# UCL/gp_emulator

Hardware: AMD Instinct MI355X
Metric: test-points/sec for predict(mean+var+grad), N_train=250 D=11 (higher is better)
Workload: dtype f64

## Files before the change

### gp_emulator_amd/csrc/gp_predict_kernel.hpp

```cpp
#pragma once
#include <hip/hip_runtime.h>
#include <stdint.h>
#include <type_traits>
#include <utility>

namespace gpk {

#ifndef GP_WAVES
#define GP_WAVES 8
#endif
#ifndef GP_WAVES_F32
#define GP_WAVES_F32 12
#endif
#ifndef GP_CHUNK
#define GP_CHUNK 64
#endif
#ifndef GP_CHUNK_F32
#define GP_CHUNK_F32 192
#endif
#ifndef GP_ABLATE
#define GP_ABLATE 0
#endif
#ifndef GP_AHEAD
#define GP_AHEAD 4
#endif
#ifndef GP_AHEAD_F32
#define GP_AHEAD_F32 8
#endif
#ifndef GP_RING_PIN
#define GP_RING_PIN 1
#endif
#ifndef GP_MU_DOUBLE
#define GP_MU_DOUBLE 1
#endif
#ifndef GP_ESTRIN
#define GP_ESTRIN 0
#endif
#ifndef GP_DOTSPLIT
#define GP_DOTSPLIT 1
#endif
#ifndef GP_GROUP_F64
#define GP_GROUP_F64 1
#endif
#ifndef GP_STAMPS
#define GP_STAMPS 0
#endif
constexpr int kTile = 16;
template <typename T, bool kVar = true> struct Geo {
  static constexpr int kWaves = sizeof(T) == 8 ? GP_WAVES : GP_WAVES_F32;
  static constexpr int kThreads = kWaves * 64;
#ifndef GP_WG_PER_CU_SMALL
#define GP_WG_PER_CU_SMALL 0
#endif
  static constexpr int kWGPerCU = kWaves >= 8 ? 1 : (GP_WG_PER_CU_SMALL > 0 ? GP_WG_PER_CU_SMALL : 8 / kWaves);
  static constexpr int kWavesPerSimd = kWaves >= 8 ? kWaves / 4 : kWGPerCU * kWaves / 4;
  static constexpr int kRowsPerWG = kWaves * kTile;
  static constexpr int kChunk = sizeof(T) == 8 ? GP_CHUNK : GP_CHUNK_F32;
};
#ifndef GP_MG_WAVES
#define GP_MG_WAVES 12
#endif
#ifndef GP_MG_WAVES_F32
#define GP_MG_WAVES_F32 16
#endif
#ifndef GP_MG_WG_PER_CU
#define GP_MG_WG_PER_CU 1
#endif
template <typename T> struct Geo<T, false> {
  static constexpr int kWaves = sizeof(T) == 8 ? GP_MG_WAVES : GP_MG_WAVES_F32;
  static constexpr int kThreads = kWaves * 64;
  static constexpr int kWGPerCU = GP_MG_WG_PER_CU;
  static constexpr int kWavesPerSimd = kWGPerCU * kWaves / 4;
  static constexpr int kRowsPerWG = kWaves * kTile;
  static constexpr int kChunk = 1;
};

typedef double f64x4 __attribute__((ext_vector_type(4)));
typedef float f32x4 __attribute__((ext_vector_type(4)));

template <typename F, int... Is>
__device__ __forceinline__ void static_for_impl(F&& f, std::integer_sequence<int, Is...>) {
  (f(std::integral_constant<int, Is>{}), ...);
}
template <int N, typename F>
__device__ __forceinline__ void static_for(F&& f) {
  static_for_impl(f, std::make_integer_sequence<int, N>{});
}

template <typename T> struct Real;
template <> struct Real<double> {
  typedef f64x4 acc_t;
  static constexpr bool kExpand = true;
  static constexpr int kGroup = GP_GROUP_F64;
  __host__ __device__ static constexpr int own_sub(int r, int g) { return 4 * r + g; }
  __device__ static inline acc_t mfma(double a, double b, acc_t c) {
    return __builtin_amdgcn_mfma_f64_16x16x4f64(a, b, c, 0, 0, 0);
  }
  __device__ static inline double exp_(double x) {
    x = __builtin_fmax(x, -1000.0);
    const double n = __builtin_rint(x * 1.4426950408889634);
    double r = fma(n, -6.93147180559945286e-01, x);
    r = fma(n, -2.31904681384629956e-17, r);
#if GP_ESTRIN
    const double r2 = r * r;
    const double p01 = fma(1.00000000000000666e+00, r, 1.0);
    const double p23 = fma(1.66666666665544028e-01, r, 5.00000000000000555e-01);
    const double p45 = fma(8.33333338566834801e-03, r, 4.16666666665732183e-02);
    const double p67 = fma(1.98411702695461072e-04, r, 1.38888889324666632e-03);
    const double p89 = fma(2.76401812311866076e-06, r, 2.48015043709117912e-05);
    const double r4 = r2 * r2;
    const double q0 = fma(r2, p23, p01);
    const double q1 = fma(r2, p67, p45);
    const double q2 = fma(r2, 2.76263485910095559e-07, p89);
    const double r8 = r4 * r4;
    const double s0 = fma(r4, q1, q0);
    const double p = fma(r8, q2, s0);
#else
    double p = 2.76263485910095559e-07;
    p = fma(p, r, 2.76401812311866076e-06);
    p = fma(p, r, 2.48015043709117912e-05);
    p = fma(p, r, 1.98411702695461072e-04);
    p = fma(p, r, 1.38888889324666632e-03);
    p = fma(p, r, 8.33333338566834801e-03);
    p = fma(p, r, 4.16666666665732183e-02);
    p = fma(p, r, 1.66666666665544028e-01);
    p = fma(p, r, 5.00000000000000555e-01);
    p = fma(p, r, 1.00000000000000666e+00);
    p = fma(p, r, 1.0);
#endif
    return ldexp(p, (int)n);
  }
  template <int GP>
  __device__ static inline void exp_n(double (&x)[GP]) {
    double n[GP], r[GP], p[GP];
#pragma unroll
    for (int u = 0; u < GP; ++u) x[u] = __builtin_fmax(x[u], -1000.0);
#pragma unroll
    for (int u = 0; u < GP; ++u) n[u] = __builtin_rint(x[u] * 1.4426950408889634);
#pragma unroll
    for (int u = 0; u < GP; ++u) r[u] = fma(n[u], -6.93147180559945286e-01, x[u]);
#pragma unroll
    for (int u = 0; u < GP; ++u) r[u] = fma(n[u], -2.31904681384629956e-17, r[u]);
#pragma unroll
    for (int u = 0; u < GP; ++u) p[u] = 2.76263485910095559e-07;
    constexpr double c[10] = {2.76401812311866076e-06, 2.48015043709117912e-05, 1.98411702695461072e-04,
                              1.38888889324666632e-03, 8.33333338566834801e-03, 4.16666666665732183e-02,
                              1.66666666665544028e-01, 5.00000000000000555e-01, 1.00000000000000666e+00, 1.0};
#pragma unroll
    for (int j = 0; j < 10; ++j) {
#pragma unroll
      for (int u = 0; u < GP; ++u) p[u] = fma(p[u], r[u], c[j]);
    }
#pragma unroll
    for (int u = 0; u < GP; ++u) x[u] = ldexp(p[u], (int)n[u]);
  }
};
template <> struct Real<float> {
  typedef f32x4 acc_t;
  static constexpr bool kExpand = false;
#ifndef GP_GROUP_F32
#define GP_GROUP_F32 2
#endif
  static constexpr int kGroup = GP_GROUP_F32;
  __host__ __device__ static constexpr int own_sub(int r, int g) { return 4 * g + r; }
  __device__ static inline acc_t mfma(float a, float b, acc_t c) {
    return __builtin_amdgcn_mfma_f32_16x16x4f32(a, b, c, 0, 0, 0);
  }
  __device__ static inline float exp_(float x) { return __expf(x); }
  template <int GP>
  __device__ static inline void exp_n(float (&x)[GP]) {
#pragma unroll
    for (int u = 0; u < GP; ++u) x[u] = __expf(x[u]);
  }
};

template <typename T>
__host__ __device__ constexpr int own_index(int I, int s, int g) {
  return 16 * I + Real<T>::own_sub(s, g);
}

template <typename T>
__host__ __device__ constexpr int point_slot(int n) {
  return 16 * (n / 16) + Real<T>::own_sub((n % 16) / 4, n % 4);
}
template <typename T>
__host__ __device__ constexpr int slot_point(int slot) {
  for (int q = 0; q < 16; ++q)
    if (Real<T>::own_sub(q / 4, q % 4) == slot % 16) return 16 * (slot / 16) + q;
  return -1;
}

struct FragId { int I, J, s; };
__host__ __device__ constexpr int frag_count(int NB) { return NB * (NB + 1) / 2 * 4; }
__host__ __device__ constexpr int frag_col_offset(int J, int NB) { return J * NB - J * (J - 1) / 2; }
__host__ __device__ constexpr FragId frag_at(int n, int NB) {
  const int pair = n >> 2;
  int J = 0;
  while (J + 1 < NB && frag_col_offset(J + 1, NB) <= pair) ++J;
  return FragId{J + pair - frag_col_offset(J, NB), J, n & 3};
}
__host__ __device__ constexpr int frag_index(int I, int J, int s, int NB) {
  return (frag_col_offset(J, NB) + (I - J)) * 4 + s;
}
__host__ __device__ constexpr int frag_count_padded(int NB, int chunk) {
  return (frag_count(NB) + chunk - 1) / chunk * chunk;
}

__host__ __device__ constexpr int row_stride(int D) { return (D + 2 + 3) & ~3; }
#ifndef GP_XA_PAD
#define GP_XA_PAD 1
#endif
template <typename T> __host__ __device__ constexpr int xa_lds_stride(int D) {
  return (GP_XA_PAD && sizeof(T) == 4 && row_stride(D) % 16 == 0) ? row_stride(D) + 4 : row_stride(D);
}

template <typename T>
struct PredictArgs {
  const T* xa;
  const T* frags;
  const T* sd;
  const T* testing;
  T* mu;
  T* var;
  T* deriv;
  long long M;
  int d_actual;
  int deriv_row_major;
  int n_emulators;
  long long xa_stride, frags_stride, sd_stride;
  unsigned long long* dbg;
  int rows_prescaled;
};

template <int XOR>
__device__ __forceinline__ unsigned swap_halves(unsigned x, unsigned& other) {
  if constexpr (XOR == 16) {
    auto r = __builtin_amdgcn_permlane16_swap(x, x, false, false);
    other = r[1];
    return r[0];
  } else {
    auto r = __builtin_amdgcn_permlane32_swap(x, x, false, false);
    other = r[1];
    return r[0];
  }
}
template <int XOR>
__device__ __forceinline__ float pair_sum(float v) {
  unsigned o, a = swap_halves<XOR>(__float_as_uint(v), o);
  return __uint_as_float(a) + __uint_as_float(o);
}
template <int XOR>
__device__ __forceinline__ double pair_sum(double v) {
  const unsigned long long u = (unsigned long long)__double_as_longlong(v);
  unsigned lo_o, hi_o;
  const unsigned lo_a = swap_halves<XOR>((unsigned)u, lo_o);
  const unsigned hi_a = swap_halves<XOR>((unsigned)(u >> 32), hi_o);
  const double a = __longlong_as_double((long long)(((unsigned long long)hi_a << 32) | lo_a));
  const double o = __longlong_as_double((long long)(((unsigned long long)hi_o << 32) | lo_o));
  return a + o;
}

template <typename T, int N>
__device__ inline void xor_reduce_groups_n(T* v) {
#pragma unroll
  for (int i = 0; i < N; ++i) v[i] = pair_sum<32>(pair_sum<16>(v[i]));
}

template <typename T>
__device__ inline T xor_reduce_groups(T v) {
  return pair_sum<32>(pair_sum<16>(v));
}

template <typename T, int kWaves = Geo<T>::kWaves, int kChunk = Geo<T>::kChunk>
__device__ __forceinline__ void stage_chunk(const T* src, T* dst, int wave, int lane) {
  constexpr int kBytes = kChunk * 64 * (int)sizeof(T);
  constexpr int kPieces = kBytes / 1024;
  static_assert(kPieces * 1024 == kBytes, "chunk must be whole 1 KiB pieces");
  const unsigned voff = (unsigned)lane * 16u;
  const unsigned lds0 = (unsigned)(uintptr_t)(
      (__attribute__((address_space(3))) char*)(reinterpret_cast<char*>(dst)));
#pragma unroll
  for (int pc0 = 0; pc0 < kPieces; pc0 += kWaves) {
    const int pc = pc0 + wave;
    if (pc0 + kWaves <= kPieces || pc < kPieces) {
      const char* s = reinterpret_cast<const char*>(src) + pc * 1024;
      const unsigned m0v = __builtin_amdgcn_readfirstlane(lds0 + pc * 1024);
      unsigned keep;
      asm volatile(
          "s_mov_b32 %0, m0\n\t"
          "s_mov_b32 m0, %1\n\t"
          "s_nop 4\n\t"
          "global_load_lds_dwordx4 %2, %3\n\t"
          "s_mov_b32 m0, %0"
          : "=&s"(keep)
          : "s"(m0v), "v"(voff), "s"(s)
          : "memory");
    }
  }
}
template <typename T, int NP>
__device__ __forceinline__ void stage_pieces(const T* src, T* dst, int first_piece, int lane) {
  const unsigned voff = (unsigned)lane * 16u;
  const unsigned lds0 = (unsigned)(uintptr_t)(
      (__attribute__((address_space(3))) char*)(reinterpret_cast<char*>(dst)));
#pragma unroll
  for (int i = 0; i < NP; ++i) {
    const int pc = first_piece + i;
    const char* s = reinterpret_cast<const char*>(src) + pc * 1024;
    const unsigned m0v = __builtin_amdgcn_readfirstlane(lds0 + pc * 1024);
    unsigned keep;
    asm volatile(
        "s_mov_b32 %0, m0\n\t"
        "s_mov_b32 m0, %1\n\t"
        "s_nop 4\n\t"
        "global_load_lds_dwordx4 %2, %3\n\t"
        "s_mov_b32 m0, %0"
        : "=&s"(keep)
        : "s"(m0v), "v"(voff), "s"(s)
        : "memory");
  }
}
__device__ __forceinline__ void dma_wait() { asm volatile("s_waitcnt vmcnt(0)" ::: "memory"); }

#if GP_STAMPS == 1
#define GP_STAMP(seg)                                                                    \
  do {                                                                                   \
    __builtin_amdgcn_sched_barrier(0);                                                   \
    unsigned long long now_;                                                             \
    asm volatile("s_memtime %0\n\ts_waitcnt lgkmcnt(0)" : "=s"(now_)::"memory");         \
    __builtin_amdgcn_sched_barrier(0);                                                   \
    seg_sum[seg] += now_ - seg_t0;                                                       \
    seg_t0 = now_;                                                                       \
  } while (0)
#else
#define GP_STAMP(seg) do { } while (0)
#endif

template <typename T, int D, int NK, bool kVar = true>
__global__ __launch_bounds__((Geo<T, kVar>::kThreads), (Geo<T, kVar>::kWavesPerSimd)) void predict_kernel(PredictArgs<T> p) {
  typedef Real<T> R;
  typedef Geo<T, kVar> G;
  constexpr int kThreads = G::kThreads;
  constexpr int kRowsPerWG = G::kRowsPerWG;
  typedef typename R::acc_t acc_t;
  constexpr int NB = (NK + 3) / 4;
  constexpr int KL = NK - 4 * (NB - 1);
  constexpr int NP = 16 * NB;
  constexpr int DSG = row_stride(D);
  constexpr int DS = xa_lds_stride<T>(D);
  constexpr int NF = frag_count(NB);
  constexpr int kChunk = G::kChunk;
  constexpr int NCH = (NF + kChunk - 1) / kChunk;

  __shared__ __attribute__((aligned(16))) T s_xa[NP * DS];
  __shared__ __attribute__((aligned(16))) T s_fr[kVar ? 2 : 1][kVar ? kChunk * 64 : 1];
  __shared__ T s_sd[2 * D + 1];
  __shared__ T s_ts[2 * D];
  __shared__ T s_rows[2][G::kWaves][kTile * D];

  const int tid = threadIdx.x;
  const int lane = tid & 63;
  const int wave = __builtin_amdgcn_readfirstlane(tid >> 6);
  const int ml = lane & 15;
  const int g = lane >> 4;

  const int n_groups = (int)((p.M + kRowsPerWG - 1) / kRowsPerWG);
  int e = 0, cur_e = -1;
  int grp = blockIdx.x;
  while (grp >= n_groups && e < p.n_emulators) { grp -= n_groups; ++e; }

  constexpr int NJ = (kTile * D + 63) / 64;
  auto fetch_rows = [&](int grp_, T (&regs)[NJ]) {
    const long long e0 = ((long long)grp_ * kRowsPerWG + wave * kTile) * p.d_actual;
    const long long emax = p.M * p.d_actual - 1;
#pragma unroll
    for (int j = 0; j < NJ; ++j) {
      long long e_ = e0 + lane + 64 * j;
      e_ = e_ < emax ? e_ : emax;
      regs[j] = p.testing[e_];
    }
  };
  auto stash_rows = [&](int buf_, const T (&regs)[NJ]) {
#pragma unroll
    for (int j = 0; j < NJ; ++j)
      if (lane + 64 * j < kTile * p.d_actual) s_rows[buf_][wave][lane + 64 * j] = regs[j];
  };
  int rbuf = 0;
  T rregs[NJ];
  if (e < p.n_emulators) {
    fetch_rows(grp, rregs);
    stash_rows(0, rregs);
  }
#if GP_STAMPS
  unsigned long long seg_sum[8] = {0, 0, 0, 0, 0, 0, 0, 0};
  unsigned long long seg_t0;
  asm volatile("s_memtime %0\n\ts_waitcnt lgkmcnt(0)" : "=s"(seg_t0)::"memory");
#endif

  for (; e < p.n_emulators;) {
    if (e != cur_e) {
      cur_e = e;
      __syncthreads();
      const T* xa = p.xa + e * p.xa_stride;
      for (int i = tid; i < NP * DSG; i += kThreads) s_xa[(i / DSG) * DS + i % DSG] = xa[i];
      const T* sdp = p.sd + e * p.sd_stride;
      if (tid < 2 * D + 1) {
        const bool live = tid == 2 * D || (tid % D) < p.d_actual;
        s_sd[tid] = live ? sdp[tid] : T(0);
        if (tid < 2 * D)
          s_ts[tid] = !live ? T(0) : !p.rows_prescaled ? sdp[tid] : tid < D ? T(1) : T(0);
      }
      if constexpr (!kVar) __syncthreads();
    }
    const T* frags = p.frags + e * p.frags_stride;
    T* o_mu = p.mu + e * p.M;
    T* o_der = p.deriv + e * p.M * p.d_actual;
    const long long m = (long long)grp * kRowsPerWG + wave * kTile + ml;
    const long long mc = m < p.M ? m : p.M - 1;

    if constexpr (kVar) {
      __syncthreads();
      stage_chunk<T, G::kWaves, kChunk>(frags, &s_fr[0][0], wave, lane);
    } else {
      (void)frags;
      __builtin_amdgcn_fence(__ATOMIC_ACQ_REL, "wavefront");
      __builtin_amdgcn_wave_barrier();
    }
    const T b = s_sd[2 * D];
    GP_STAMP(0);

    T t[D];
    T gm = T(0);
    {
      T sdv[D], cv[D], rv[D];
#pragma unroll
      for (int d = 0; d < D; ++d) {
        const int dc = d < p.d_actual ? d : p.d_actual - 1;
        sdv[d] = s_ts[d];
        cv[d] = s_ts[D + d];
        rv[d] = s_rows[rbuf][wave][ml * p.d_actual + dc];
      }
#pragma unroll
      for (int d = 0; d < D; ++d) {
        t[d] = sdv[d] * (rv[d] - cv[d]);
        gm = fma(t[d], t[d], gm);
      }
    }
    gm *= T(-0.5);
    const T poison = gm - gm;

    asm volatile("" :: "v"(gm));
    int e_next = e, grp_next = grp + gridDim.x;
    while (grp_next >= n_groups && e_next < p.n_emulators) { grp_next -= n_groups; ++e_next; }
    fetch_rows(e_next < p.n_emulators ? grp_next : grp, rregs);

    GP_STAMP(1);
    T kv[NK];
#if GP_MU_DOUBLE
    double mu = 0.0;
#else
    T mu = T(0);
#endif
    T ga[D];
#pragma unroll
    for (int d = 0; d < D; ++d) ga[d] = T(0);

    constexpr int GP = R::kGroup;
    static_for<(NK + GP - 1) / GP>([&](auto qc) {
      constexpr int q0 = decltype(qc)::value * GP;
      constexpr int GU = NK - q0 < GP ? NK - q0 : GP;
      T x[GP][D];
      T al[GP];
      T k[GP];
#pragma unroll
      for (int u = 0; u < GU; ++u) {
        const int q = q0 + u;
        const int i = own_index<T>(q >> 2, q & 3, g);
        const T* row = &s_xa[i * DS];
#pragma unroll
        for (int d = 0; d < D; ++d) x[u][d] = row[d];
        al[u] = row[D];
        if constexpr (R::kExpand) k[u] = row[D + 1] + gm;
      }
#pragma unroll
      for (int u = 0; u < GU; ++u) {
#if GP_ABLATE == 2
        continue;
#endif
        if constexpr (R::kExpand) {
          T part[GP_DOTSPLIT];
          part[0] = k[u];
#pragma unroll
          for (int c = 1; c < GP_DOTSPLIT; ++c) part[c] = T(0);
#pragma unroll
          for (int d = 0; d < D; ++d) part[d % GP_DOTSPLIT] = fma(x[u][d], t[d], part[d % GP_DOTSPLIT]);
#pragma unroll
          for (int c = 1; c < GP_DOTSPLIT; ++c) part[0] += part[c];
          k[u] = part[0];
        } else {
          T r2 = T(0);
#pragma unroll
          for (int d = 0; d < D; ++d) {
            x[u][d] -= t[d];
            r2 = fma(x[u][d], x[u][d], r2);
          }
          k[u] = T(-0.5) * r2;
        }
      }
#pragma unroll
      for (int u = 0; u < GU; ++u) {
#if GP_ABLATE == 2
        k[u] = x[u][0] + t[0];
#else
        k[u] = R::kExpand ? R::exp_(k[u]) : b * R::exp_(k[u]);
#endif
        if constexpr (kVar) kv[q0 + u] = k[u];
      }
#pragma unroll
      for (int u = 0; u < GU; ++u) {
        const T w = k[u] * al[u];
        mu += (decltype(mu))w;
#if GP_ABLATE == 2
        ga[u % D] += w;
#else
#pragma unroll
        for (int d = 0; d < D; ++d) ga[d] = fma(w, x[u][d], ga[d]);
#endif
      }
    });
    GP_STAMP(2);
    const T mu_t = (T)xor_reduce_groups(mu) + poison;
    static_for<(D + 5) / 6>([&](auto bc) {
      constexpr int d0 = decltype(bc)::value * 6;
      constexpr int nb_ = (D - d0 < 6) ? (D - d0) : 6;
      xor_reduce_groups_n<T, nb_>(&ga[d0]);
    });
    {
      T sdv[D];
#pragma unroll
      for (int d = 0; d < D; ++d) sdv[d] = s_sd[d];
#pragma unroll
      for (int d = 0; d < D; ++d)
        ga[d] = sdv[d] * (R::kExpand ? fma(-t[d], mu_t, ga[d]) : ga[d]);
    }

    if (m < p.M) {
      if (g == 0) o_mu[m] = mu_t;
#pragma unroll
      for (int d = 0; d < D; ++d) {
        if ((d & 3) == g && d < p.d_actual) {
          if (p.deriv_row_major) o_der[m * p.d_actual + d] = ga[d];
          else o_der[(long long)d * p.M + m] = ga[d];
        }
      }
    }

    GP_STAMP(3);
    stash_rows(rbuf ^ 1, rregs);
    if constexpr (!kVar) {
      rbuf ^= 1;
      e = e_next;
      grp = grp_next;
      continue;
    } else {

    T* o_var = p.var + e * p.M;
    T vacc = T(0);
    acc_t acc;
    constexpr int kAhead = sizeof(T) == 4 ? GP_AHEAD_F32 : GP_AHEAD;
    T afr[kAhead];
#if GP_ABLATE == 1
    static_for<NK>([&](auto qc) { vacc += kv[decltype(qc)::value]; });
    static_for<0>([&](auto fc) {
#else
    static_for<NF>([&](auto fc) {
#endif
      constexpr int f = decltype(fc)::value;
      constexpr int c = f / kChunk, fl = f % kChunk;
      constexpr FragId fid = frag_at(f, NB);
      constexpr int I = fid.I, J = fid.J, s = fid.s;
      if constexpr (fl == 0) {
#if GP_ABLATE == 4
        if constexpr (c == 0) { dma_wait(); __syncthreads(); }
#else
        dma_wait();
        __syncthreads();
        if constexpr (c + 1 < NCH)
          stage_chunk<T>(frags + (c + 1) * kChunk * 64, &s_fr[(c + 1) & 1][0], wave, lane);
#endif
        static_for<kAhead - 1>([&](auto jc) {
          constexpr int j = decltype(jc)::value;
#if GP_ABLATE >= 3
          if constexpr (j < kChunk && f + j < NF) afr[j % kAhead] = kv[j % NK];
#else
          if constexpr (j < kChunk && f + j < NF) afr[j % kAhead] = s_fr[c & 1][j * 64 + lane];
#endif
        });
      }
#if GP_ABLATE >= 3
      if constexpr (fl + kAhead - 1 < kChunk && f + kAhead - 1 < NF)
        afr[(fl + kAhead - 1) % kAhead] = kv[(f + 1) % NK];
#else
      if constexpr (fl + kAhead - 1 < kChunk && f + kAhead - 1 < NF)
        afr[(fl + kAhead - 1) % kAhead] = s_fr[c & 1][(fl + kAhead - 1) * 64 + lane];
#endif
      if constexpr (I == J && s == 0) acc = acc_t{T(0), T(0), T(0), T(0)};
      if constexpr (4 * I + s < NK) acc = R::mfma(afr[fl % kAhead], kv[4 * I + s], acc);
#if GP_RING_PIN
      if constexpr (sizeof(T) == 4 || GP_RING_PIN > 1) __builtin_amdgcn_sched_barrier(0);
#endif
      if constexpr (I == NB - 1 && s == 3) {
#pragma unroll
        for (int r = 0; r < (J == NB - 1 ? KL : 4); ++r) vacc = fma(acc[r], kv[4 * J + r], vacc);
      }
    });
    rbuf ^= 1;
    GP_STAMP(4);
    vacc = xor_reduce_groups(vacc);
    if (m < p.M && g == 1) o_var[m] = b - vacc + poison;

    e = e_next;
    grp = grp_next;
    GP_STAMP(5);
    }
  }
#if GP_STAMPS
  if (lane == 0 && p.dbg) {
    for (int k_ = 0; k_ < 8; ++k_) atomicAdd(&p.dbg[k_], seg_sum[k_]);
    atomicAdd(&p.dbg[7], 1ull);
  }
#endif
}

}
```

Before: 746.3 million.

## Triple-buffer fragment staging with deeper lookahead and branch-free derivative stores

Makes the LDS fragment ring buffer configurable, with a default of three buffers for f64 when the LDS budget allows. This stages chunks further ahead, so fewer chunk boundaries have to wait on the DMA and barrier, and the afr prefetch is allowed to cross chunk boundaries. The derivative write loop is also reworked into per-group select-then-store with a hidden group index, which replaces the predicated per-d branches. The cost is more LDS use, which may reduce occupancy, plus more complex barrier and schedule pinning.

```diff
diff --git a/gp_emulator_amd/csrc/gp_predict_kernel.hpp b/gp_emulator_amd/csrc/gp_predict_kernel.hpp
--- a/gp_emulator_amd/csrc/gp_predict_kernel.hpp
+++ b/gp_emulator_amd/csrc/gp_predict_kernel.hpp
@@ -214,6 +214,26 @@
   return (GP_XA_PAD && sizeof(T) == 4 && row_stride(D) % 16 == 0) ? row_stride(D) + 4 : row_stride(D);
 }
 
+#ifndef GP_FRAG_BUFS
+#define GP_FRAG_BUFS 3
+#endif
+#ifndef GP_FRAG_BUFS_F32
+#define GP_FRAG_BUFS_F32 2
+#endif
+constexpr int kLdsBudget = 160 * 1024;
+constexpr int kLdsSlack = 32;
+template <typename T>
+__host__ __device__ constexpr int predict_lds_bytes(int D, int NK, int bufs) {
+  const int NP = 16 * ((NK + 3) / 4);
+  return (int)sizeof(T) * (NP * xa_lds_stride<T>(D) + bufs * Geo<T>::kChunk * 64 + (2 * D + 1) + 2 * D +
+                           2 * Geo<T>::kWaves * kTile * D) + kLdsSlack;
+}
+template <typename T>
+__host__ __device__ constexpr int frag_buffers(int D, int NK) {
+  const int want = sizeof(T) == 8 ? GP_FRAG_BUFS : GP_FRAG_BUFS_F32;
+  return want > 2 && predict_lds_bytes<T>(D, NK, want) <= kLdsBudget ? want : 2;
+}
+
 template <typename T>
 struct PredictArgs {
   const T* xa;
@@ -351,12 +371,16 @@
   constexpr int NF = frag_count(NB);
   constexpr int kChunk = G::kChunk;
   constexpr int NCH = (NF + kChunk - 1) / kChunk;
+  constexpr int kBufs = kVar ? frag_buffers<T>(D, NK) : 1;
+  constexpr int kLook = kBufs - 2;
 
   __shared__ __attribute__((aligned(16))) T s_xa[NP * DS];
-  __shared__ __attribute__((aligned(16))) T s_fr[kVar ? 2 : 1][kVar ? kChunk * 64 : 1];
+  __shared__ __attribute__((aligned(16))) T s_fr[kBufs][kVar ? kChunk * 64 : 1];
   __shared__ T s_sd[2 * D + 1];
   __shared__ T s_ts[2 * D];
   __shared__ T s_rows[2][G::kWaves][kTile * D];
+  static_assert(!kVar || (int)(sizeof(s_xa) + sizeof(s_fr) + sizeof(s_sd) + sizeof(s_ts) + sizeof(s_rows)) + kLdsSlack ==
+                             predict_lds_bytes<T>(D, NK, kBufs), "predict_lds_bytes() does not count the kernel's LDS arrays");
 
   const int tid = threadIdx.x;
   const int lane = tid & 63;
@@ -381,6 +405,8 @@
     }
   };
   auto stash_rows = [&](int buf_, const T (&regs)[NJ]) {
+#pragma unroll
+    for (int j = 0; j < NJ; ++j) asm volatile("" ::"v"(regs[j]));
 #pragma unroll
     for (int j = 0; j < NJ; ++j)
       if (lane + 64 * j < kTile * p.d_actual) s_rows[buf_][wave][lane + 64 * j] = regs[j];
@@ -420,7 +446,10 @@
 
     if constexpr (kVar) {
       __syncthreads();
-      stage_chunk<T, G::kWaves, kChunk>(frags, &s_fr[0][0], wave, lane);
+      static_for<1 + kLook>([&](auto cc) {
+        constexpr int c = decltype(cc)::value;
+        if constexpr (c < NCH) stage_chunk<T, G::kWaves, kChunk>(frags + c * kChunk * 64, &s_fr[c][0], wave, lane);
+      });
     } else {
       (void)frags;
       __builtin_amdgcn_fence(__ATOMIC_ACQ_REL, "wavefront");
@@ -546,12 +575,26 @@
 
     if (m < p.M) {
       if (g == 0) o_mu[m] = mu_t;
-#pragma unroll
-      for (int d = 0; d < D; ++d) {
-        if ((d & 3) == g && d < p.d_actual) {
-          if (p.deriv_row_major) o_der[m * p.d_actual + d] = ga[d];
-          else o_der[(long long)d * p.M + m] = ga[d];
-        }
+      int gs = g;
+      asm volatile("" : "+v"(gs));
+      T gq[(D + 3) / 4];
+#pragma unroll
+      for (int q = 0; q < (D + 3) / 4; ++q) {
+        gq[q] = ga[4 * q];
+#pragma unroll
+        for (int u = 1; u < 4; ++u)
+          if (4 * q + u < D) gq[q] = gs == u ? ga[4 * q + u] : gq[q];
+      }
+      if (p.deriv_row_major) {
+        T* o_row = o_der + m * p.d_actual + gs;
+#pragma unroll
+        for (int q = 0; q < (D + 3) / 4; ++q)
+          if (4 * q + gs < p.d_actual) o_row[4 * q] = gq[q];
+      } else {
+        T* o_row = o_der + gs * p.M + m;
+#pragma unroll
+        for (int q = 0; q < (D + 3) / 4; ++q)
+          if (4 * q + gs < p.d_actual) o_row[4 * q * p.M] = gq[q];
       }
     }
 
@@ -583,29 +626,43 @@
 #if GP_ABLATE == 4
         if constexpr (c == 0) { dma_wait(); __syncthreads(); }
 #else
-        dma_wait();
-        __syncthreads();
-        if constexpr (c + 1 < NCH)
-          stage_chunk<T>(frags + (c + 1) * kChunk * 64, &s_fr[(c + 1) & 1][0], wave, lane);
+        if constexpr (c == 0 || c + kLook < NCH) {
+          dma_wait();
+          if constexpr (kLook > 0) {
+            if constexpr (c > 0) __builtin_amdgcn_sched_barrier(0);
+            asm volatile("s_barrier" ::: "memory");
+            if constexpr (c > 0) __builtin_amdgcn_sched_barrier(0);
+          } else {
+            __syncthreads();
+          }
+          if constexpr (c + kLook + 1 < NCH)
+            stage_chunk<T, G::kWaves, kChunk>(frags + (c + kLook + 1) * kChunk * 64,
+                                              &s_fr[(c + kLook + 1) % kBufs][0], wave, lane);
+        }
 #endif
         static_for<kAhead - 1>([&](auto jc) {
-          constexpr int j = decltype(jc)::value;
+          constexpr int n = f + decltype(jc)::value;
+          if constexpr (n < NF && (c == 0 || n / kChunk > c - 1 + kLook)) {
 #if GP_ABLATE >= 3
-          if constexpr (j < kChunk && f + j < NF) afr[j % kAhead] = kv[j % NK];
-#else
-          if constexpr (j < kChunk && f + j < NF) afr[j % kAhead] = s_fr[c & 1][j * 64 + lane];
-#endif
+            afr[n % kAhead] = kv[n % NK];
+#else
+            afr[n % kAhead] = s_fr[(n / kChunk) % kBufs][(n % kChunk) * 64 + lane];
+#endif
+          }
         });
       }
+      {
+        constexpr int n = f + kAhead - 1;
+        if constexpr (n < NF && n / kChunk <= c + kLook) {
 #if GP_ABLATE >= 3
-      if constexpr (fl + kAhead - 1 < kChunk && f + kAhead - 1 < NF)
-        afr[(fl + kAhead - 1) % kAhead] = kv[(f + 1) % NK];
-#else
-      if constexpr (fl + kAhead - 1 < kChunk && f + kAhead - 1 < NF)
-        afr[(fl + kAhead - 1) % kAhead] = s_fr[c & 1][(fl + kAhead - 1) * 64 + lane];
-#endif
+          afr[n % kAhead] = kv[(f + 1) % NK];
+#else
+          afr[n % kAhead] = s_fr[(n / kChunk) % kBufs][(n % kChunk) * 64 + lane];
+#endif
+        }
+      }
       if constexpr (I == J && s == 0) acc = acc_t{T(0), T(0), T(0), T(0)};
-      if constexpr (4 * I + s < NK) acc = R::mfma(afr[fl % kAhead], kv[4 * I + s], acc);
+      if constexpr (4 * I + s < NK) acc = R::mfma(afr[f % kAhead], kv[4 * I + s], acc);
 #if GP_RING_PIN
       if constexpr (sizeof(T) == 4 || GP_RING_PIN > 1) __builtin_amdgcn_sched_barrier(0);
 #endif
```

Result: faster. 759.3 million (median of 6 runs) (+1.7%).
